# slothfulxtx/Texture-GS

Hardware: AMD Instinct MI355X
Metric: fwd+bwd views/sec @800x800, 300k Gaussians + 1024^2 texture; HBM GB/s vs roofline (higher is better)
Workload: dtype f32; 1 GPU; c3: N=300000 Gaussians, cubemap 6x1024x1024x3 f32, 800x800, fwd+bwd, sh_degree 3; parallelism=views sharded dp1, view_pipeline=3 HIP streams, order=accumulate, forwards begun one view per stream ahead, grad_allreduce=none (1 GPU)

## Files before the change

### include/texgs.h

```cpp
#ifndef TEXGS_H
#define TEXGS_H

#include <stddef.h>
#include <stdint.h>

#ifdef __cplusplus
extern "C" {
#endif

#define TEXGS_ABI_VERSION 19
#define TEXGS_TILE 16
#define TEXGS_REC_TEST_FLOATS 8
#define TEXGS_REC_SHADE_FLOATS 20
#define TEXGS_ACC_FLOATS 32

typedef struct TexGSFrame {
    int32_t image_height;
    int32_t image_width;
    float   tanfovx;
    float   tanfovy;
    float   scale_modifier;
    int32_t sh_degree;
    int32_t sh_coeffs;
    int32_t tex_res;
// ... 33 lines not shown
typedef struct TexGSBinning {
    uint32_t  num_rendered;
    uint64_t* keys_unsorted;
    uint64_t* keys_sorted;
    uint32_t* point_list;
    uint32_t* ranges;
    uint32_t* tile_order;
    void*     sort_temp;
    size_t    sort_temp_bytes;
} TexGSBinning;

typedef struct TexGSImage {
    float*    out_color;
    float*    out_depth;
    float*    out_norm;
    float*    out_alpha;
    float*    final_T;
    uint32_t* n_contrib;
    uint32_t* tex_bin_count;
    uint32_t* survivors;
    uint16_t* surv_qmask;
    uint32_t* surv_count;
    uint32_t* tex_bin_resv;
} TexGSImage;
#define TEXGS_RESV_WORDS 192

#define TEXGS_ACC_MEANS3D 1
#define TEXGS_ACC_MEANS2D 2
#define TEXGS_ACC_SHS 4
#define TEXGS_ACC_OPACITIES 8
#define TEXGS_ACC_SCALES 16
#define TEXGS_ACC_ROTATIONS 32
#define TEXGS_ACC_UVS 64
#define TEXGS_ACC_COLOR_OFFSET 128
#define TEXGS_ACC_COV3D 256
#define TEXGS_ACC_ALL 511

#define TEXGS_WANT_TEXTURE   1
#define TEXGS_WANT_GAUSSIANS 2
#define TEXGS_WANT_ALL       3

typedef struct TexGSGrads {
    const float* dL_dcolor;
    const float* dL_ddepth;
    const float* dL_dnorm;
    const float* dL_dalpha;
    float* acc;
    float* dL_dmeans3D;
// ... 190 lines not shown
```

### texture-gs_amd/csrc/render.hip

```cpp
#include "common.h"
#include "wave_ops.h"
#include "texrec_math.h"

namespace {

typedef unsigned long long ull;

struct __attribute__((packed, aligned(4))) Texel3 { float x, y, z; };
__device__ __forceinline__ Texel3 load_texel(const float* __restrict__ tex, uint32_t boff) {
    return *reinterpret_cast<const Texel3*>(reinterpret_cast<const char*>(tex) + boff);
}

typedef uint32_t tg_u4 __attribute__((ext_vector_type(4)));
template <class T> __device__ __forceinline__ T nt_load(const T* p) {
    return __builtin_nontemporal_load(p);
}
template <class T> __device__ __forceinline__ void nt_store(T* p, T v) {
    __builtin_nontemporal_store(v, p);
}
__device__ __forceinline__ uint2 nt_load2(const uint2* p) {
    const unsigned long long v = nt_load(reinterpret_cast<const unsigned long long*>(p));
    return make_uint2((uint32_t)v, (uint32_t)(v >> 32));
}
__device__ __forceinline__ void nt_store2(uint2* p, uint2 v) {
// ... 53 lines not shown
        return ah * dx * dx + bh * dx * dy + ch * dy * dy;
    };
    auto edge_y = [&](float dy) {
        const float dx = fminf(dx1, fmaxf(dx0, bh * dy * iha));
        return ah * dx * dx + bh * dx * dy + ch * dy * dy;
    };
    const float best = fmaxf(fmaxf(edge_x(dx0), edge_x(dx1)), fmaxf(edge_y(dy0), edge_y(dy1)));
    return best >= thr - 1e-3f * fabsf(thr) - 1e-4f;
}

struct PixArgs {
    int W, H, tiles_x, num_tiles, R;
    const uint2* ranges;
    const uint32_t* tile_order;
    const uint32_t* point_list;
    const float4* rec_test;
    const float4* rec_shade;
    const float* texture;
    const float* bg;
    uint2*    surv;
    uint16_t* surv_qm;
    uint32_t* surv_cnt;
    uint32_t* resv;
};

__device__ __forceinline__ bool wave_block(const PixArgs& a, int& tile, int& wave) {
    const int b = (int)blockIdx.x, k = b >> 3;
    wave = k & 3;
    const int rank = ((k >> 2) << 3) | (b & 7);
    if (rank >= a.num_tiles) return false;
    tile = (int)a.tile_order[rank];
    return true;
}
inline int blend_grid(int num_tiles) { return 4 * ((num_tiles + 7) & ~7); }

#define TG_BALLOT(P) __builtin_amdgcn_ballot_w64((bool)(P))
__device__ __forceinline__ int mbcnt64(ull m) {
    return (int)__builtin_amdgcn_mbcnt_hi((uint32_t)(m >> 32), __builtin_amdgcn_mbcnt_lo((uint32_t)m, 0u));
}

__device__ __forceinline__ uint32_t tap_bin(const CubeTap& ct, int nb) { return (uint32_t)((ct.face * nb + (ct.y0 >> 5)) * nb + (ct.x0 >> 5)); }
__device__ __forceinline__ bool tap_binned(const CubeTap& ct) { return ct.dox != 0u && ct.doy != 0u; }
#define TG_RESV 64
#define TG_RESV_EMPTY 0xFFFFFFFFu
#define TG_SLOT_NONE 0xFFFFFFFFu
#define TG_SLOT_OVF  0x80000000u
__device__ __forceinline__ int tap_home(const CubeTap& ct) { return ((ct.x0 >> 5) & 7) | (((ct.y0 >> 5) & 7) << 3); }
template <class P> __device__ __forceinline__ uint32_t& resv_bin(P& p, int h) { return reinterpret_cast<uint32_t*>(&p.B[h])[3]; }

#define TG_RING 128
#define TG_DUMMY 64
struct Planes {
    float4 A[65];
    float4 B[65];
    float4 C[65];
    float4 D[65];
    float4 E[65];
    float4 F[65];
    float2 G[66];
};

#define KEY_J(K)   ((int)((K) & 127u))
#define KEY_PL(K)  ((int)(((K) >> 8) & 63u))
#define KEY_OX(K)  ((int)(((K) >> 14) & 7u))
#define KEY_OY(K)  ((int)(((K) >> 17) & 7u))

__device__ __forceinline__ void lane_pixel(int lane, int& ox, int& oy) {
    ox = (((lane >> 4) & 1) << 2) | (lane & 3);
    oy = (((lane >> 5) & 1) << 2) | ((lane >> 2) & 3);
}

__device__ __forceinline__ void load_chunk(const PixArgs& a, Planes& P, int lane, bool live, uint32_t id, uint32_t pos,
                                           float4& T0, float4& T1) {
    const float4 z = make_float4(0.f, 0.f, 0.f, 0.f);
    float4 S0 = z, S1 = z, S2 = z, S3 = z, S4 = z;
    T0 = z; T1 = make_float4(0.f, 0.f, -1.f, 1.f);
    if (live) {
        const float4* __restrict__ tp = a.rec_test + 2 * (size_t)id;
        const float4* __restrict__ sp = a.rec_shade + (TEXGS_REC_SHADE_FLOATS / 4) * (size_t)id;
        T0 = tp[0]; T1 = tp[1]; S0 = sp[0]; S1 = sp[1]; S2 = sp[2]; S3 = sp[3]; S4 = sp[4];
    }
    P.A[lane] = T0;
    { float* pb = reinterpret_cast<float*>(&P.B[lane]); pb[0] = T1.x; pb[1] = T1.y; pb[2] = __uint_as_float(pos); }
    P.C[lane] = make_float4(S3.z, S3.w, S4.x, S4.y);
    P.D[lane] = S0; P.E[lane] = S1; P.F[lane] = S2;
    P.G[lane] = make_float2(S3.x, S3.y);
}
__device__ __forceinline__ void init_dummy(Planes& P, int lane) {
    if (lane == 0) {
        const float4 z = make_float4(0.f, 0.f, 0.f, 0.f);
        P.A[TG_DUMMY] = z; P.B[TG_DUMMY] = make_float4(0.f, 0.f, __uint_as_float(0xFFFFFFFFu), 0.f); P.C[TG_DUMMY] = z;
        P.D[TG_DUMMY] = z; P.E[TG_DUMMY] = z; P.F[TG_DUMMY] = z; P.G[TG_DUMMY] = make_float2(0.f, 0.f);
    }
}

#define FQ_CAP 128
struct __attribute__((aligned(16))) FwdLds {
    Planes p;
    uint2 q[FQ_CAP];
    ull col[64 * 3];
    uint32_t ring[TG_RING];
    uint8_t list[4][64];
    uint32_t ccnt[TG_RESV / 2];
// ... 127 lines not shown
            const float4 t0 = nt0, t1 = nt1;
            r += 64;
            nt0 = zt0; nt1 = zt1;
            if (r + lane < todo) {
                const float4* __restrict__ tp = a.rec_test + 2 * (size_t)nid;
                nt0 = tp[0]; nt1 = tp[1];
            }
            nid = (r + 64 + lane < todo) ? a.point_list[range.x + r + 64 + lane] : 0u;
            const bool reach = block_reachable(t0.x, t0.y, t0.z, t0.w, t1.x, t1.w, t1.z, wpx, wpy, 7.0f);
            const ull m = TG_BALLOT(reach);
            if (reach) L.ring[(qh + nq + mbcnt64(m)) & (TG_RING - 1)] = (uint32_t)idx;
            nq += __popcll(m);
        }
        if (nq == 0) break;
        const int take = min(64, nq);
        __builtin_amdgcn_wave_barrier();
        uint32_t pos = 0xFFFFFFFFu, id = 0u;
        if (lane < take) {
            pos = L.ring[(qh + lane) & (TG_RING - 1)];
            id = a.point_list[range.x + pos];
        }
        qh = (qh + take) & (TG_RING - 1); nq -= take;
        float4 T0, T1;
        load_chunk(a, L.p, lane, lane < take, id, pos, T0, T1);
        reinterpret_cast<uint32_t*>(&L.list[0][0])[lane] = 0x40404040u;
        __builtin_amdgcn_wave_barrier();
        int len[4];
        uint32_t qbits = 0u;
#pragma unroll
        for (int q = 0; q < 4; ++q) {
            const bool rowdone = ((done_mask >> (16 * q)) & 0xFFFFull) == 0xFFFFull;
            const bool geo = (lane < take) &&
                block_reachable(T0.x, T0.y, T0.z, T0.w, T1.x, T1.w, T1.z, wpx + (float)((q & 1) << 2), wpy + (float)((q >> 1) << 2), 3.0f);
            qbits |= geo ? (1u << q) : 0u;
            const bool rq = geo && !rowdone;
            const ull m = TG_BALLOT(rq);
            len[q] = __popcll(m);
            if (rq) L.list[q][mbcnt64(m)] = (uint8_t)lane;
        }
        if (a.surv != nullptr) {
            if (lane < take) { nt_store2(a.surv + sbase + nsurv + lane, make_uint2(id, pos)); nt_store(a.surv_qm + sbase + nsurv + lane, (uint16_t)qbits); }
            nsurv += take;
        }
        __builtin_amdgcn_wave_barrier();
        int tmax = max(max(len[0], len[1]), max(len[2], len[3]));
        auto test_one = [&](const float4& A, const float4& B, const float4& Cc, const int j) -> bool {
                const float power = gauss_power(A.z, A.w, B.x, A.x - pxf, A.y - pyf);
// ... 105 lines not shown
using texrec_math::rec_word0;
using texrec_math::rec_pack;
using texrec_math::rec_unpack;
__device__ __forceinline__ void rec_store(uint32_t* __restrict__ base, uint32_t slot, const Rec4 r) {
    tg_u4 v; v.x = r.a; v.y = r.b; v.z = r.c; v.w = r.d;
    __builtin_nontemporal_store(v, reinterpret_cast<tg_u4*>(base) + slot);
}
__device__ __forceinline__ Rec4 rec_load(const Rec4* __restrict__ p) {
    const tg_u4 v = __builtin_nontemporal_load(reinterpret_cast<const tg_u4*>(p));
    Rec4 r; r.a = v.x; r.b = v.y; r.c = v.z; r.d = v.w;
    return r;
}

#define TG_MOMENTS_ALL  0x0FFFFFFFu
#define TG_MOMENTS_NOUV (0x3Fu | (0x7Fu << 21))

#ifdef K7_TRACE
#define K7_TRACE_BLOCKS 32768
__device__ unsigned long long k7_trace[4 * K7_TRACE_BLOCKS];
#endif
namespace k7_occ {
#define BQ_CAP 64
#define K7_GATHER 1
#define K7_WAVES_PER_SIMD 4
#include "render_bwd_body.h"
#undef BQ_CAP
#undef K7_GATHER
#undef K7_WAVES_PER_SIMD
}
namespace k7_lds {
#define BQ_CAP 128
#define K7_GATHER 0
#define K7_WAVES_PER_SIMD 2
#include "render_bwd_body.h"
#undef BQ_CAP
#undef K7_GATHER
#undef K7_WAVES_PER_SIMD
}

__global__ void __launch_bounds__(1024)
k_bin_offsets(int nbins, const uint32_t* __restrict__ count, uint32_t* __restrict__ base, uint32_t* __restrict__ cursor,
              uint32_t* __restrict__ order, uint32_t* __restrict__ stats) {
    constexpr int BO_MAX = 32;
    __shared__ uint32_t s_w[16];
    __shared__ uint32_t s_carry;
    const int tid = (int)threadIdx.x, lane = tid & 63, wv = tid >> 6;
    if (tid == 0) s_carry = 0u;
    __syncthreads();
    for (int c0 = 0; c0 < nbins; c0 += 1024 * BO_MAX) {
        const int n = min(nbins - c0, 1024 * BO_MAX);
        const int per = (n + 1023) >> 10;
        const int i0 = c0 + tid * per;
        uint32_t v[BO_MAX];
        uint32_t sum = 0u;
#pragma unroll
        for (int k = 0; k < BO_MAX; ++k) { v[k] = (k < per && i0 + k < c0 + n) ? count[i0 + k] + count[nbins + i0 + k] : 0u; sum += v[k]; }
        uint32_t incl = sum;
#pragma unroll
        for (int d = 1; d < 64; d <<= 1) { const uint32_t o = (uint32_t)__shfl_up((int)incl, d, 64); if (lane >= d) incl += o; }
// ... 99 lines not shown
            if (y >= R || xq >= R * 3) continue;
            unsafeAtomicAdd(dtex + ((size_t)(face * R + y) * R) * 3 + xq, texrec_math::from_fixed(q, down));
        }
        __syncthreads();
    }
}

inline PixArgs make_pix(const CamConst& c, const TexGSFrame* f, const TexGSInputs* in, const TexGSGeom* g,
                        const TexGSBinning* b, const TexGSImage* img) {
    PixArgs a;
    a.W = c.W; a.H = c.H; a.tiles_x = c.tiles_x; a.num_tiles = c.tiles_x * c.tiles_y; a.R = c.R;
    a.ranges = reinterpret_cast<const uint2*>(b->ranges);
    a.point_list = b->point_list;
    a.tile_order = b->tile_order;
    a.rec_test = reinterpret_cast<const float4*>(g->rec_test);
    a.rec_shade = reinterpret_cast<const float4*>(g->rec_shade);
    a.texture = in->texture;
    a.bg = f->bg;
    const bool hand = img->survivors != nullptr && img->surv_qmask != nullptr && img->surv_count != nullptr;
    a.surv = hand ? reinterpret_cast<uint2*>(img->survivors) : nullptr;
    a.surv_qm = hand ? img->surv_qmask : nullptr;
    a.surv_cnt = hand ? img->surv_count : nullptr;
    a.resv = img->tex_bin_resv;
    return a;
}

inline TexBinArgs make_bins(const CamConst& c, const TexGSImage* img, const TexGSGrads* gr) {
    TexBinArgs tb;
    tb.nb = (c.R + 31) >> 5;
    const bool on = (gr->want & TEXGS_WANT_TEXTURE) && img->tex_bin_count != nullptr && img->tex_bin_resv != nullptr && gr->tex_bins != nullptr &&
                    gr->tex_bin_cursor != nullptr && gr->tex_bin_base != nullptr && gr->tex_rec_cap > 0;
    tb.rec = on ? reinterpret_cast<uint32_t*>(gr->tex_bins) : nullptr;
    tb.cursor = on ? gr->tex_bin_cursor : nullptr;
    tb.base = on ? gr->tex_bin_base : nullptr;
    tb.order = on ? gr->tex_bin_base + tex_bin_count(c.R) + 1 : nullptr;
    tb.stats = on ? gr->tex_bin_cursor + tex_bin_count(c.R) : nullptr;
    tb.cap = on ? gr->tex_rec_cap : 0u;
    return tb;
}

}

size_t tex_bin_count(int R) {
    const size_t nb = (size_t)((R + 31) >> 5);
    return 6 * nb * nb;
}
// ... 4 lines not shown
    if (in->texture)
        hipLaunchKernelGGL(k_render_fwd<true>, dim3(blend_grid(a.num_tiles)), dim3(64), 0, s, a, img->out_color, img->out_depth,
                           img->out_norm, img->out_alpha, img->final_T, img->n_contrib, img->tex_bin_resv ? img->tex_bin_count : (uint32_t*)nullptr);
    else
        hipLaunchKernelGGL(k_render_fwd<false>, dim3(blend_grid(a.num_tiles)), dim3(64), 0, s, a, img->out_color, img->out_depth,
                           img->out_norm, img->out_alpha, img->final_T, img->n_contrib, (uint32_t*)nullptr);
    return hipGetLastError();
}

hipError_t launch_render_bwd(const CamConst& c, const TexGSFrame* f, const TexGSInputs* in, const TexGSGeom* g,
                       const TexGSBinning* b, const TexGSImage* img, TexGSGrads* gr, hipStream_t s) {
    const PixArgs a = make_pix(c, f, in, g, b, img);
    const TexBinArgs tb = make_bins(c, img, gr);
    const bool taps = in->texture != nullptr;
    const bool tex = taps && (gr->want & TEXGS_WANT_TEXTURE) && gr->dL_dtexture != nullptr;
    const bool geo = (gr->want & TEXGS_WANT_GAUSSIANS) != 0;
    if (!tex && !geo) return hipSuccess;
    if (tex && tb.rec)
        hipLaunchKernelGGL(k_bin_offsets, dim3(1), dim3(1024), 0, s, (int)tex_bin_count(c.R), (const uint32_t*)img->tex_bin_count,
                           gr->tex_bin_base, gr->tex_bin_cursor, gr->tex_bin_base + tex_bin_count(c.R) + 1, tb.stats);
    const dim3 grid(blend_grid(a.num_tiles)), blk(64);
#define K7_LAUNCH(NS, TEX, GEO, UVG, TAPS) hipLaunchKernelGGL((NS::k_render_bwd<TEX, GEO, UVG, TAPS>), grid, blk, 0, s, a, tb, img->final_T, \
        img->n_contrib, gr->dL_dcolor, gr->dL_ddepth, gr->dL_dnorm, gr->dL_dalpha, gr->acc, gr->dL_dtexture)
    if (!taps)            K7_LAUNCH(k7_occ, false, true, false, false);
    else if (tex && geo)  K7_LAUNCH(k7_occ, true, true, true, true);
    else if (tex)         K7_LAUNCH(k7_lds, true, false, false, true);
    else                  K7_LAUNCH(k7_occ, false, true, true, true);
#undef K7_LAUNCH
    return hipGetLastError();
}

bool tex_bins_enabled(const CamConst& c, const TexGSInputs* in, const TexGSImage* img, const TexGSGrads* gr) {
    return in->texture != nullptr && gr->dL_dtexture != nullptr && make_bins(c, img, gr).rec != nullptr;
}

hipError_t launch_texgrad_reduce(const CamConst& c, const TexGSImage* img, TexGSGrads* gr, hipStream_t s) {
    const TexBinArgs tb = make_bins(c, img, gr);
    if (!tb.rec) return hipSuccess;
    hipLaunchKernelGGL(k_texgrad_reduce, dim3((unsigned)tex_bin_count(c.R)), dim3(TB_THREADS), 0, s, c.R, tb, gr->dL_dtexture);
    return hipGetLastError();
}

#ifdef K7_TRACE
extern "C" __attribute__((visibility("default"))) int texgs_debug_k7_trace(void* host_dst) {
    return (int)hipMemcpyFromSymbol(host_dst, HIP_SYMBOL(k7_trace), sizeof(unsigned long long) * 4 * K7_TRACE_BLOCKS);
}
#endif
```

### texture-gs_amd/csrc/render_bwd_body.h

```cpp
#if K7_GATHER
struct PlanesT { float4 A[65]; float4 B[65]; };
#else
typedef Planes PlanesT;
#endif
struct __attribute__((aligned(16))) BwdLds {
    float4 items[BQ_CAP * 3 + 3];
    float4 abuf[BQ_CAP];
    PlanesT p;
    float4 dpix[64];
    float4 dgeo[64];
    uint32_t task[64];
    uint8_t list[4][64];
    uint32_t tpos[TG_RESV], tend[TG_RESV];
};

template <bool TEX, bool GEO, bool UVG, bool TAPS>
__global__ void __launch_bounds__(64, K7_WAVES_PER_SIMD)
k_render_bwd(PixArgs a, TexBinArgs tb, const float* __restrict__ final_T, const uint32_t* __restrict__ n_contrib,
             const float* __restrict__ dL_dcolor, const float* __restrict__ dL_ddepth,
             const float* __restrict__ dL_dnorm, const float* __restrict__ dL_dalpha,
             float* __restrict__ acc, float* __restrict__ dtex) {
    static_assert(TAPS || (!TEX && !UVG), "no texture: no texture gradient and no UV chain");
    static_assert(GEO || !UVG, "the UV chain ends in the per-Gaussian moments");
    static_assert(TEX || GEO, "nothing to compute");
// ... 67 lines not shown
    uint2 nsv = make_uint2(0u, 0xFFFFFFFFu);
    uint32_t nqm = 0u;
    if (ns - 1 - lane >= 0) { nsv = nt_load2(a.surv + sbase + (ns - 1 - lane)); nqm = nt_load(a.surv_qm + sbase + (ns - 1 - lane)); }
    struct Seg { int n_items, n_it; uint32_t it_lo, it_hi, it_first; };
    struct Round {
        bool have;
        int e, pl, jj, axis;
        uint32_t key;
        uint32_t slot;
        uint32_t ovf0, ovf1;
        uint32_t fxw, fyw;
        uint32_t o00, dox, doy;
        float w, vd0, vd1, vd2, nu0, nu1, nu2, inv;
        float T, araw;
        float fx, fy, ka, kb, kc, kd;
        Texel3 t00, t01, t10, t11;
#if K7_GATHER
        float4 sd, se, sf;
        float4 c5;
#endif
    };
    uint32_t cid = 0u;
    (void)cid;
    auto front_a = [&](int rbase, Round& R, int n_items) {
        R.e = rbase + lane;
        R.have = R.e < n_items;
        float4 it = make_float4(1.f, 0.f, 0.f, 0.f);
        if (R.have) {
            it = L.abuf[R.e];
        }
        R.key = __float_as_uint(it.w);
        R.pl = KEY_PL(R.key);
        R.jj = KEY_J(R.key);
        if constexpr (GEO) { R.T = it.x; R.araw = it.z; }
        else R.w = fminf(TG_ALPHA_MAX, it.z) * it.x;
#if K7_GATHER
        const float4* __restrict__ sp = a.rec_shade + (TEXGS_REC_SHADE_FLOATS / 4) * (size_t)(uint32_t)__builtin_amdgcn_ds_bpermute(R.jj << 2, (int)cid);
        if constexpr (TAPS) { R.sd = sp[0]; R.se = sp[1]; }
        R.sf = sp[2];
        const float4 s3 = sp[3];
        const float2 s4 = *reinterpret_cast<const float2*>(sp + 4);
        R.vd1 = s3.x; R.vd2 = s3.y;
        R.c5 = make_float4(s3.z, s3.w, s4.x, s4.y);
#endif
    };
    auto front_b = [&](Round& R) {
        const uint32_t key = R.key;
        const int jj = R.jj;
#if K7_GATHER
        const float4 f_ = R.sf;
        R.vd0 = f_.w;
#else
        const float4 f_ = L.p.F[jj];
        const float2 g2 = L.p.G[jj];
        R.vd0 = f_.w; R.vd1 = g2.x; R.vd2 = g2.y;
#endif
        if constexpr (TAPS) {
            const float2 xy = *reinterpret_cast<const float2*>(&L.p.A[jj]);
#if K7_GATHER
            const float4 d_ = R.sd, e4 = R.se;
// ... 99 lines not shown
                const uint32_t p1 = (uint32_t)__builtin_amdgcn_ds_bpermute(ldr, (int)R.ovf1);
                if (ovf) { const uint32_t pos = p0 + (slot & 63u); slot = (pos < p1) ? pos : TG_SLOT_NONE; }
            }
            if (slot < tb.cap) {
                rec_store(tb.rec, slot, rec_pack(R.fxw, R.fyw >> 10, (int)(R.fyw & 31u), (int)((R.fyw >> 5) & 31u), x0, x1, x2));
            } else if (R.have && (x0 != 0.f || x1 != 0.f || x2 != 0.f)) {
                scatter_direct(dtex, R.o00, R.dox, R.doy, R.fx, R.fy, x0, x1, x2);
            }
        }
    };
    for (int hi = ns; hi > 0; hi -= 64) {
        if (hi > 128) __builtin_amdgcn_s_setprio(3); else if (hi > 64) __builtin_amdgcn_s_setprio(2); else __builtin_amdgcn_s_setprio(0);
        const bool live = hi - 1 - lane >= 0;
        const uint32_t id = nsv.x, pos = nsv.y, qm = nqm;
        nsv = make_uint2(0u, 0xFFFFFFFFu); nqm = 0u;
        if (hi - 65 - lane >= 0) { nsv = nt_load2(a.surv + sbase + (hi - 65 - lane)); nqm = nt_load(a.surv_qm + sbase + (hi - 65 - lane)); }
        const int take = min(64, hi);
        if ((int)__builtin_amdgcn_readlane((int)pos, take - 1) >= wave_last) continue;
        __builtin_amdgcn_wave_barrier();
        cid = id;
#if K7_GATHER
        {
            float4 T0 = make_float4(0.f, 0.f, 0.f, 0.f), T1 = make_float4(0.f, 0.f, -1.f, 1.f);
            if (live) { const float4* __restrict__ tp = a.rec_test + 2 * (size_t)id; T0 = tp[0]; T1 = tp[1]; }
            L.p.A[lane] = T0;
            float* pb = reinterpret_cast<float*>(&L.p.B[lane]); pb[0] = T1.x; pb[1] = T1.y; pb[2] = __uint_as_float(pos);
        }
#else
        float4 T0, T1;
        load_chunk(a, L.p, lane, live, id, pos, T0, T1);
#endif
        reinterpret_cast<uint32_t*>(&L.list[0][0])[lane] = 0x40404040u;
        __builtin_amdgcn_wave_barrier();
        int len[4];
#pragma unroll
        for (int q = 0; q < 4; ++q) {
            const bool rq = live && ((int)pos < rowlast[q]) && ((qm >> q) & 1u);
            const ull m = TG_BALLOT(rq);
            len[q] = __popcll(m);
            if (rq) L.list[q][mbcnt64(m)] = (uint8_t)lane;
        }
        __builtin_amdgcn_wave_barrier();
        const int tmax = max(max(len[0], len[1]), max(len[2], len[3]));
        int t = 0;
        auto stage_a = [&](Seg& sg) {
            sg.n_it = 0; sg.n_items = 0; sg.it_lo = 0u; sg.it_hi = 0u; sg.it_first = 0u;
            auto test_one = [&](const float4& cA, const float4& cB, const int cj) -> bool {
// ... 186 lines not shown
```

### texture-gs_amd/texgs/_lib.py

```python
import contextlib
import ctypes as C
import os

_HERE = os.path.dirname(os.path.abspath(__file__))
LIB_PATH = os.environ.get("TEXGS_LIB") or os.path.join(os.path.dirname(_HERE), "libtexgs.so")

ABI_VERSION = 19
TILE = 16
REC_TEST_FLOATS = 8
REC_SHADE_FLOATS = 20
TEXBIN_RECORD_FLOATS = 4
RESV_WORDS = 192
ACC_FLOATS = 32
WANT_TEXTURE, WANT_GAUSSIANS, WANT_ALL = 1, 2, 3

_fp = C.c_void_p


class Frame(C.Structure):
    _fields_ = [("image_height", C.c_int32), ("image_width", C.c_int32), ("tanfovx", C.c_float),
                ("tanfovy", C.c_float), ("scale_modifier", C.c_float), ("sh_degree", C.c_int32),
                ("sh_coeffs", C.c_int32), ("tex_res", C.c_int32), ("num_gaussians", C.c_int32),
                ("debug", C.c_int32), ("bg", _fp), ("viewmatrix", _fp), ("projmatrix", _fp), ("campos", _fp)]


class Inputs(C.Structure):
    _fields_ = [("means3D", _fp), ("shs", _fp), ("opacities", _fp), ("scales", _fp), ("rotations", _fp),
                ("uvs", _fp), ("gradient_uvs", _fp), ("texture", _fp), ("color_offset", _fp), ("cov3D_precomp", _fp)]


class Geom(C.Structure):
    _fields_ = [("rec_test", _fp), ("rec_shade", _fp), ("depth", _fp), ("radii", _fp), ("rect", _fp), ("tiles_touched", _fp),
                ("offsets", _fp), ("scan_temp", _fp), ("scan_temp_bytes", C.c_size_t)]


class Binning(C.Structure):
    _fields_ = [("num_rendered", C.c_uint32), ("keys_unsorted", _fp), ("keys_sorted", _fp), ("point_list", _fp),
                ("ranges", _fp), ("tile_order", _fp), ("sort_temp", _fp), ("sort_temp_bytes", C.c_size_t)]


class Image(C.Structure):
    _fields_ = [("out_color", _fp), ("out_depth", _fp), ("out_norm", _fp), ("out_alpha", _fp),
                ("final_T", _fp), ("n_contrib", _fp), ("tex_bin_count", _fp),
                ("survivors", _fp), ("surv_qmask", _fp), ("surv_count", _fp), ("tex_bin_resv", _fp)]


class Grads(C.Structure):
    _fields_ = [("dL_dcolor", _fp), ("dL_ddepth", _fp), ("dL_dnorm", _fp), ("dL_dalpha", _fp), ("acc", _fp),
                ("dL_dmeans3D", _fp), ("dL_dmeans2D", _fp), ("dL_dshs", _fp), ("dL_dopacities", _fp),
                ("dL_dscales", _fp), ("dL_drotations", _fp), ("dL_duvs", _fp), ("dL_dtexture", _fp),
                ("dL_dcolor_offset", _fp), ("dL_dcov3D", _fp), ("want", C.c_uint32), ("tex_bins", _fp), ("tex_bin_cursor", _fp), ("tex_bin_base", _fp),
                ("tex_rec_cap", C.c_uint32),
                ("accumulate", C.c_int32), ("dL_dvd_residue", _fp)]


class UVNetStruct(C.Structure):
    _fields_ = [(n, _fp) for n in ("W1", "b1", "W2", "b2", "emb", "W3", "b3", "W4", "b4", "W5", "b5", "xyz_offset", "xyz_scale")] \
        + [("hidden", C.c_int32)]


class HashGridStruct(C.Structure):
    _fields_ = [("n_levels", C.c_int32), ("n_features", C.c_int32), ("log2_hashmap_size", C.c_int32), ("base_resolution", C.c_float),
                ("per_level_scale", C.c_float)]


HASHGRID_MAX_LEVELS = 16
HASHGRID_FEATURES = 4
# ... 184 lines not shown
```

### texture-gs_amd/texgs/rasterizer.py

```python
import ctypes as C
import math
import os as _os
import threading as _threading
import weakref as _weakref
from collections import namedtuple
from types import SimpleNamespace
from typing import NamedTuple

import torch
from torch import nn

from . import _lib

USE_TEX_BINS = _os.environ.get("TEXGS_TEX_BINS", "1") != "0"
TEX_REC_CAP = int(_os.environ.get("TEXGS_REC_CAP", "0"))
DIRECT_LEAF_GRADS = _os.environ.get("TEXGS_DIRECT_LEAF_GRADS", "0") != "0"
TEX_REC_BYTES_MAX = int(float(_os.environ.get("TEXGS_BIN_GB_MAX", "4")) * (1 << 30))
_ACC_BITS = dict(means3D=1, means2D=2, shs=4, opacities=8, scales=16, rotations=32, uvs=64, color_offset=128, cov3D=256)


class GaussianRasterizationSettings(NamedTuple):
    image_height: int
    image_width: int
    tanfovx: float
    tanfovy: float
    bg: torch.Tensor
    scale_modifier: float
    viewmatrix: torch.Tensor
    projmatrix: torch.Tensor
    sh_degree: int
    campos: torch.Tensor
    prefiltered: bool
    debug: bool


_ptr = _lib.ptr


def _f32c(t: torch.Tensor, name: str, device) -> torch.Tensor:
    if not isinstance(t, torch.Tensor):
# ... 203 lines not shown
def _pin_take(words):
    pool = _PIN_POOL.setdefault(words, [])
    return pool.pop() if pool else torch.empty(max(words, 1), dtype=torch.int32).pin_memory()


def _pin_give(t):
    pool = _PIN_POOL.setdefault(t.numel(), [])
    if len(pool) < 16:
        pool.append(t)


def _prefetch_take(device, key):
    skey = (device.index, int(torch.cuda.current_stream(device).cuda_stream))
    lst = _PREFETCH.get(skey, ())
    for k, (key_k, fwd) in enumerate(lst):
        if key_k == key:
            del lst[k]
            if not lst:
                del _PREFETCH[skey]
            return fwd


_Args = namedtuple("_Args", "means3D shs opacities scales rotations uvs gradient_uvs texture color_offset cov3D_precomp N K R")
_HANDOFF = tuple(n for n, _ in _lib.Image._fields_[6:])


def _check_inputs(st, means3D, shs, opacities, scales, rotations, uvs, gradient_uvs, texture, color_offset=None, cov3D_precomp=None):
    device = means3D.device
    N = means3D.shape[0]
    means3D = _f32c(means3D, "means3D", device)
    if means3D.dim() != 2 or means3D.shape[1] != 3:
        raise ValueError("means3D must be [N,3]")
    opacities = _f32c(opacities, "opacities", device)
    if opacities.numel() != N:
        raise ValueError(f"per-Gaussian inputs must have exactly N rows (N={N}; opacities {tuple(opacities.shape)})")
    if cov3D_precomp is not None:
        if texture is not None:
            raise ValueError("cov3D_precomp is an input of the untextured surface only")
        cov3D_precomp = _f32c(cov3D_precomp, "cov3D_precomp", device)
        if cov3D_precomp.shape != (N, 6):
            raise ValueError(f"cov3D_precomp must be [N,6], got {tuple(cov3D_precomp.shape)}")
        scales = rotations = None
    else:
        scales = _f32c(scales, "scales", device)
        rotations = _f32c(rotations, "rotations", device)
        if scales.shape != (N, 3) or rotations.shape != (N, 4):
            raise ValueError("per-Gaussian inputs must have exactly N rows "
# ... 19 lines not shown
        K = shs.shape[1]
        if K > 15:
            raise ValueError("shs holds at most 15 view-dependent coefficients (degree 3)")
    if color_offset is not None:
        color_offset = _f32c(color_offset, "color_offset", device)
        if color_offset.shape != (N, 3):
            raise ValueError(f"color_offset must be [N,3], got {tuple(color_offset.shape)}")
    if int(st.sh_degree) < 0 or int(st.sh_degree) > 3:
        raise ValueError("sh_degree must be in [0,3]")
    return _Args(means3D, shs, opacities, scales, rotations, uvs, gradient_uvs, texture, color_offset, cov3D_precomp, N, K, R)


def _add_handoff(ar, cap, tiles, R, want_counts):
    if cap is not None:
        ar.add("survivors", (4 * max(cap, 1), 2), torch.int32)
        ar.add("surv_qmask", (4 * max(cap, 1),), torch.int16)
    if tiles is not None:
        ar.add("surv_count", (4 * tiles,), torch.int32)
        if want_counts:
            ar.add("tex_bin_count", (2 * int(_lib.load().texgs_tex_bin_count(R)),), torch.int32)
            ar.add("tex_bin_resv", (4 * tiles, _lib.RESV_WORDS), torch.int32)


class _Forward:

    def __init__(self, st, tensors, for_backward, count_bins, lazy):
        self.st, self.raw, self.flags = st, tensors, (for_backward, count_bins, lazy)

    def key(self):
        t = lambda x: None if x is None else (x.data_ptr(), x._version, tuple(x.shape), x.requires_grad)
        st = self.st
        return (int(st.image_height), int(st.image_width), float(st.tanfovx), float(st.tanfovy), float(st.scale_modifier), int(st.sh_degree),
                bool(st.debug), t(st.bg), t(st.viewmatrix), t(st.projmatrix), t(st.campos)) + tuple(t(x) for x in self.raw) + self.flags

    def begin(self):
        lib = _lib.load()
        self._plan()
        a, N, stream = self.args, self.args.N, self.stream
        with torch.cuda.device(a.means3D.device):
            self.fix.commit()
            self._bind()
            refs = self.refs
            _lib.call(lib.texgs_preprocess_forward, *refs, stream)
            pin = self.pin = _pin_take(int(lib.texgs_num_rendered_words(N)))
            _lib.call(lib.texgs_num_rendered_begin, refs[2], N, pin.data_ptr(), pin.numel(), 0, stream)
            self.d_ev = torch.cuda.Event()
# ... 60 lines not shown
        self.binning = self.bin_ar = None
        if entry is None and not batched:
            self._alloc_bin(self.cap, fix)
        self.refs = [C.byref(x) for x in (self.frame, self.inputs, self.geom)]

    def _add_lists(self, ar):
        ar.add("ranges", (self.tiles, 2), torch.int32)
        ar.add("tile_order", (self.tiles,), torch.int32)
        if self.handoff:
            _add_handoff(ar, None, self.tiles, self.args.R, self.want_counts)

    def _alloc_bin(self, cap, lists_ar, commit=True):
        c1, tiles = max(cap, 1), self.tiles
        sort_bytes = _lib.load().texgs_sort_temp_bytes(cap, tiles)
        ar = self.bin_ar = _Arena(self.fix.device)
        ar.add("keys_unsorted", (c1,), torch.int64)
        ar.add("keys_sorted", (c1,), torch.int64)
        ar.add("point_list", (c1,), torch.int32)
        ar.add("sort_temp", (sort_bytes,), torch.uint8)
        if lists_ar is None:
            self._add_lists(ar)
        if self.handoff:
            _add_handoff(ar, cap, None, self.args.R, self.want_counts)
        self.sort_bytes = sort_bytes
        if commit:
            ar.commit()
            self._bind_bin(lists_ar)
        return ar

    def _bind_bin(self, lists_ar):
        ar, sort_bytes = self.bin_ar, self.sort_bytes
        la = lists_ar if lists_ar is not None else ar
        self.binning = _lib.Binning(0, ar.ptr("keys_unsorted"), ar.ptr("keys_sorted"), ar.ptr("point_list"), la.ptr("ranges"),
                                    la.ptr("tile_order"), ar.ptr("sort_temp"), sort_bytes)
        for n in _HANDOFF:
            setattr(self.img, n, (ar if n in ar.specs else la).ptr(n))

    def finish(self):
        lib, a, img, entry, refs = _lib.load(), self.args, self.img, self.entry, self.refs
        for_backward, _, lazy = self.flags
        stream, cap, pin = self.stream, self.cap, self.pin
        if self.binned is not None:
            D, fp, ready = self.binned
            shared, binning = False, self.binning
            with torch.cuda.device(a.means3D.device):
                cur = torch.cuda.current_stream(a.means3D.device)
                if cur.cuda_stream != stream:
                    cur.wait_event(ready)
                from .multiview import views_entries
                _lib.call(views_entries().render_forward_binned, *refs, C.byref(binning), C.byref(img), cur.cuda_stream)
            return self._finished(binning, D, cap, shared, fp)
        with torch.cuda.device(a.means3D.device):
            self.d_ev.synchronize()
            d_host, fp_host = C.c_uint32(0), C.c_uint64(0)
            _lib.call(lib.texgs_num_rendered_reduce, pin.data_ptr(), a.N, C.byref(d_host), C.byref(fp_host))
            _pin_give(pin)
            D, fp = int(d_host.value), int(fp_host.value)
            shared = entry is not None and fp == entry.fingerprint and D == entry.D
            if shared:
# ... 9 lines not shown
                if entry is not None:
                    cap = max(cap, grown)
                    self._alloc_bin(cap, None)
                    _lib.call(lib.texgs_depth_sort_scan, refs[2], a.N, stream)
                elif D > cap:
                    cap = grown
                    self._alloc_bin(cap, self.fix)
                binning = self.binning
                binning.num_rendered = D
                _lib.call(lib.texgs_bin_sort_render_forward, *refs, C.byref(binning), C.byref(img), stream)
                _CAPACITY_HINT[self.hint_key] = max(_CAPACITY_HINT.get(self.hint_key, 0), grown)
                if GEOM_CACHE:
                    _GEOM[self.gkey] = _GeomEntry(
                        self.gints, self.cam_key, fp, D, cap, tuple(getattr(binning, n) for n, _ in _lib.Binning._fields_[1:]),
                        (self.fix, self.bin_ar), (img.survivors, img.surv_qmask, img.surv_count) if self.handoff else None,
                        (img.tex_bin_count, img.tex_bin_resv) if (self.handoff and img.tex_bin_count) else None)
        return self._finished(binning, D, cap, shared, fp)

    def _finished(self, binning, D, cap, shared, fp):
        a, img, entry = self.args, self.img, self.entry
        for_backward, _, lazy = self.flags
        arenas = (self.fix,) + ((self.bin_ar,) if self.bin_ar is not None else ()) + (tuple(entry.arenas) if shared else ())
        tensors = _Tensors(arenas, keep=self.keep, radii=self.outs[4], for_backward=bool(for_backward))
        for n in _HANDOFF:
            if getattr(img, n) is None:
                tensors[n] = None
        state = _State(self.frame, self.inputs, self.geom, binning, img, tensors, a, D, cap, self.tiles, self.want_counts,
                       bool(lazy and for_backward), shared)
        state.fingerprint = fp
        return self.outs, state

    def abandon(self):
        if self.binned is not None:
            return
        self.d_ev.synchronize()
        _pin_give(self.pin)


_BATCH_SCOPE = None


class _Request:
    __slots__ = ("fwd", "stream", "batched")

    def __init__(self, fwd, stream):
        self.fwd, self.stream, self.batched = fwd, stream, False

# ... 156 lines not shown
    fwd = _Forward(st, (means3D, shs, opacities, scales, rotations, uvs, gradient_uvs, texture, color_offset, cov3D_precomp),
                   for_backward, count_bins, lazy)
    if _BATCH_SCOPE is not None:
        _BATCH_SCOPE.requests.append(_Request(fwd, torch.cuda.current_stream(device)))
        return
    _register_begun(fwd.begin(), limit=4)


def forward_raw(st, means3D, shs, opacities, scales, rotations, uvs, gradient_uvs, texture, color_offset=None,
                for_backward=True, cov3D_precomp=None, count_bins=None, lazy=False):
    _gpu_only(means3D.device)
    fwd = _Forward(st, (means3D, shs, opacities, scales, rotations, uvs, gradient_uvs, texture, color_offset, cov3D_precomp),
                   for_backward, count_bins, lazy)
    pend = _prefetch_take(means3D.device, fwd.key()) if _PREFETCH else None
    return (pend or fwd.begin()).finish()


def _late_handoff(s: _State):
    lib = _lib.load()
    device = s.args.means3D.device
    stream = torch.cuda.current_stream(device).cuda_stream
    ar = _Arena(device)
    _add_handoff(ar, s.cap, s.tiles, s.R, s.want_counts)
    ar.add("scratch_out", (8, s.H, s.W), torch.float32)
    ar.add("final_T", (s.H, s.W), torch.float32)
    ar.add("n_contrib", (s.H, s.W), torch.int32)
    ar.commit()
    so = ar.ptr("scratch_out")
    hw = 4 * s.H * s.W
    img = _lib.Image(so, so + 3 * hw, so + 4 * hw, so + 7 * hw, ar.ptr("final_T"), ar.ptr("n_contrib"), *(ar.ptr(n) for n in _HANDOFF))
    _lib.call(lib.texgs_render_forward, C.byref(s.frame), C.byref(s.inputs), C.byref(s.geom), C.byref(s.bin), C.byref(img), stream)
    s.tensors._arenas = tuple(s.tensors._arenas) + (ar,)
    for n in _HANDOFF:
        setattr(s.img, n, ar.ptr(n))
        s.tensors.pop(n, None)
        if n not in ar.specs:
            s.tensors[n] = None
    _GEOM_STATS["late_handoffs"] += 1


def _plan_outputs(N, K, textured, has_cov, has_coff, want, sinks, device):
    shapes = {}
    if want & _lib.WANT_GAUSSIANS:
        shapes = dict(means3D=(N, 3), means2D=(N, 3), opacities=(N, 1))
        if has_cov:
            shapes["cov3D"] = (N, 6)
        else:
            shapes.update(scales=(N, 3), rotations=(N, 4))
        if textured:
            shapes["uvs"] = (N, 3)
        if K > 0:
            shapes["shs"] = (N, K, 3)
        if has_coff:
            shapes["color_offset"] = (N, 3)
    fresh = [n for n in shapes if n not in sinks]
    sizes = [math.prod(shapes[n]) for n in fresh]
    flat = torch.empty(sum(sizes), dtype=torch.float32, device=device).split(sizes) if fresh else ()
    outs, mask = {n: v.view(shapes[n]) for n, v in zip(fresh, flat)}, 0
    for n in shapes.keys() - set(fresh):
        t = outs[n] = sinks[n]
# ... 227 lines not shown
```

Before: 1070 views/s.

## Stream survivor Gaussian records from forward to backward as contiguous rows

```diff
diff --git a/include/texgs.h b/include/texgs.h
--- a/include/texgs.h
+++ b/include/texgs.h
@@ -79,8 +79,10 @@
     uint16_t* surv_qmask;
     uint32_t* surv_count;
     uint32_t* tex_bin_resv;
+    float*    surv_rec;
 } TexGSImage;
 #define TEXGS_RESV_WORDS 192
+#define TEXGS_SURV_ROW_FLOATS 24
 
 #define TEXGS_ACC_MEANS3D 1
 #define TEXGS_ACC_MEANS2D 2
diff --git a/texture-gs_amd/csrc/render.hip b/texture-gs_amd/csrc/render.hip
--- a/texture-gs_amd/csrc/render.hip
+++ b/texture-gs_amd/csrc/render.hip
@@ -99,6 +99,7 @@
     uint16_t* surv_qm;
     uint32_t* surv_cnt;
     uint32_t* resv;
+    float4*   surv_rec;
 };
 
 __device__ __forceinline__ bool wave_block(const PixArgs& a, int& tile, int& wave) {
@@ -136,6 +137,12 @@
     float4 F[65];
     float2 G[66];
 };
+#define TG_SURV_ROW (TEXGS_SURV_ROW_FLOATS / 4)
+static_assert(TEXGS_SURV_ROW_FLOATS == 24, "surv_row_store and K7's row offsets state the 96-byte row");
+__device__ __forceinline__ void surv_row_store(float4* __restrict__ row, const float4& T0, const float4& T1, const float4& S0,
+                                               const float4& S1, const float4& S2, const float4& S3, const float4& S4) {
+    row[0] = T0; row[1] = S0; row[2] = S1; row[3] = S2; row[4] = S3; row[5] = make_float4(S4.x, S4.y, T1.x, T1.y);
+}
 
 #define KEY_J(K)   ((int)((K) & 127u))
 #define KEY_PL(K)  ((int)(((K) >> 8) & 63u))
@@ -148,7 +155,7 @@
 }
 
 __device__ __forceinline__ void load_chunk(const PixArgs& a, Planes& P, int lane, bool live, uint32_t id, uint32_t pos,
-                                           float4& T0, float4& T1) {
+                                           float4& T0, float4& T1, float4* __restrict__ row = nullptr) {
     const float4 z = make_float4(0.f, 0.f, 0.f, 0.f);
     float4 S0 = z, S1 = z, S2 = z, S3 = z, S4 = z;
     T0 = z; T1 = make_float4(0.f, 0.f, -1.f, 1.f);
@@ -156,6 +163,7 @@
         const float4* __restrict__ tp = a.rec_test + 2 * (size_t)id;
         const float4* __restrict__ sp = a.rec_shade + (TEXGS_REC_SHADE_FLOATS / 4) * (size_t)id;
         T0 = tp[0]; T1 = tp[1]; S0 = sp[0]; S1 = sp[1]; S2 = sp[2]; S3 = sp[3]; S4 = sp[4];
+        if (row != nullptr) surv_row_store(row, T0, T1, S0, S1, S2, S3, S4);
     }
     P.A[lane] = T0;
     { float* pb = reinterpret_cast<float*>(&P.B[lane]); pb[0] = T1.x; pb[1] = T1.y; pb[2] = __uint_as_float(pos); }
@@ -329,7 +337,8 @@
         }
         qh = (qh + take) & (TG_RING - 1); nq -= take;
         float4 T0, T1;
-        load_chunk(a, L.p, lane, lane < take, id, pos, T0, T1);
+        load_chunk(a, L.p, lane, lane < take, id, pos, T0, T1,
+                   a.surv_rec != nullptr ? a.surv_rec + TG_SURV_ROW * (sbase + (size_t)(nsurv + lane)) : nullptr);
         reinterpret_cast<uint32_t*>(&L.list[0][0])[lane] = 0x40404040u;
         __builtin_amdgcn_wave_barrier();
         int len[4];
@@ -481,19 +490,34 @@
 namespace k7_occ {
 #define BQ_CAP 64
 #define K7_GATHER 1
+#define K7_STREAM 0
 #define K7_WAVES_PER_SIMD 4
 #include "render_bwd_body.h"
 #undef BQ_CAP
 #undef K7_GATHER
+#undef K7_STREAM
+#undef K7_WAVES_PER_SIMD
+}
+namespace k7_str {
+#define BQ_CAP 64
+#define K7_GATHER 1
+#define K7_STREAM 1
+#define K7_WAVES_PER_SIMD 4
+#include "render_bwd_body.h"
+#undef BQ_CAP
+#undef K7_GATHER
+#undef K7_STREAM
 #undef K7_WAVES_PER_SIMD
 }
 namespace k7_lds {
 #define BQ_CAP 128
 #define K7_GATHER 0
+#define K7_STREAM 0
 #define K7_WAVES_PER_SIMD 2
 #include "render_bwd_body.h"
 #undef BQ_CAP
 #undef K7_GATHER
+#undef K7_STREAM
 #undef K7_WAVES_PER_SIMD
 }
 
@@ -639,6 +663,7 @@
     a.surv_qm = hand ? img->surv_qmask : nullptr;
     a.surv_cnt = hand ? img->surv_count : nullptr;
     a.resv = img->tex_bin_resv;
+    a.surv_rec = hand ? reinterpret_cast<float4*>(img->surv_rec) : nullptr;
     return a;
 }
 
@@ -689,10 +714,11 @@
     const dim3 grid(blend_grid(a.num_tiles)), blk(64);
 #define K7_LAUNCH(NS, TEX, GEO, UVG, TAPS) hipLaunchKernelGGL((NS::k_render_bwd<TEX, GEO, UVG, TAPS>), grid, blk, 0, s, a, tb, img->final_T, \
         img->n_contrib, gr->dL_dcolor, gr->dL_ddepth, gr->dL_dnorm, gr->dL_dalpha, gr->acc, gr->dL_dtexture)
-    if (!taps)            K7_LAUNCH(k7_occ, false, true, false, false);
-    else if (tex && geo)  K7_LAUNCH(k7_occ, true, true, true, true);
+    const bool str = a.surv_rec != nullptr;
+    if (!taps)            { if (str) K7_LAUNCH(k7_str, false, true, false, false); else K7_LAUNCH(k7_occ, false, true, false, false); }
+    else if (tex && geo)  { if (str) K7_LAUNCH(k7_str, true, true, true, true);    else K7_LAUNCH(k7_occ, true, true, true, true); }
     else if (tex)         K7_LAUNCH(k7_lds, true, false, false, true);
-    else                  K7_LAUNCH(k7_occ, false, true, true, true);
+    else                  { if (str) K7_LAUNCH(k7_str, false, true, true, true);   else K7_LAUNCH(k7_occ, false, true, true, true); }
 #undef K7_LAUNCH
     return hipGetLastError();
 }
diff --git a/texture-gs_amd/csrc/render_bwd_body.h b/texture-gs_amd/csrc/render_bwd_body.h
--- a/texture-gs_amd/csrc/render_bwd_body.h
+++ b/texture-gs_amd/csrc/render_bwd_body.h
@@ -1,3 +1,6 @@
+#if K7_STREAM && !K7_GATHER
+#error "the survivor stream replaces the gathers of the K7_GATHER configuration"
+#endif
 #if K7_GATHER
 struct PlanesT { float4 A[65]; float4 B[65]; };
 #else
@@ -113,6 +116,10 @@
     };
     uint32_t cid = 0u;
     (void)cid;
+#if K7_STREAM
+    const char* __restrict__ srow = reinterpret_cast<const char*>(a.surv_rec + TG_SURV_ROW * sbase);
+    int chi = 0;
+#endif
     auto front_a = [&](int rbase, Round& R, int n_items) {
         R.e = rbase + lane;
         R.have = R.e < n_items;
@@ -126,7 +133,11 @@
         if constexpr (GEO) { R.T = it.x; R.araw = it.z; }
         else R.w = fminf(TG_ALPHA_MAX, it.z) * it.x;
 #if K7_GATHER
+#if K7_STREAM
+        const float4* __restrict__ sp = reinterpret_cast<const float4*>(srow + (uint32_t)(chi - 1 - R.jj) * (uint32_t)(16 * TG_SURV_ROW)) + 1;
+#else
         const float4* __restrict__ sp = a.rec_shade + (TEXGS_REC_SHADE_FLOATS / 4) * (size_t)(uint32_t)__builtin_amdgcn_ds_bpermute(R.jj << 2, (int)cid);
+#endif
         if constexpr (TAPS) { R.sd = sp[0]; R.se = sp[1]; }
         R.sf = sp[2];
         const float4 s3 = sp[3];
@@ -272,7 +283,17 @@
 #if K7_GATHER
         {
             float4 T0 = make_float4(0.f, 0.f, 0.f, 0.f), T1 = make_float4(0.f, 0.f, -1.f, 1.f);
+#if K7_STREAM
+            chi = hi;
+            if (live) {
+                const float4* __restrict__ tp = reinterpret_cast<const float4*>(srow + (uint32_t)(hi - 1 - lane) * (uint32_t)(16 * TG_SURV_ROW));
+                T0 = tp[0];
+                const float2 t1 = *reinterpret_cast<const float2*>(reinterpret_cast<const float*>(tp + TG_SURV_ROW - 1) + 2);
+                T1.x = t1.x; T1.y = t1.y;
+            }
+#else
             if (live) { const float4* __restrict__ tp = a.rec_test + 2 * (size_t)id; T0 = tp[0]; T1 = tp[1]; }
+#endif
             L.p.A[lane] = T0;
             float* pb = reinterpret_cast<float*>(&L.p.B[lane]); pb[0] = T1.x; pb[1] = T1.y; pb[2] = __uint_as_float(pos);
         }
diff --git a/texture-gs_amd/texgs/_lib.py b/texture-gs_amd/texgs/_lib.py
--- a/texture-gs_amd/texgs/_lib.py
+++ b/texture-gs_amd/texgs/_lib.py
@@ -10,6 +10,7 @@
 REC_TEST_FLOATS = 8
 REC_SHADE_FLOATS = 20
 TEXBIN_RECORD_FLOATS = 4
+SURV_ROW_FLOATS = 24
 RESV_WORDS = 192
 ACC_FLOATS = 32
 WANT_TEXTURE, WANT_GAUSSIANS, WANT_ALL = 1, 2, 3
@@ -42,7 +43,7 @@
 class Image(C.Structure):
     _fields_ = [("out_color", _fp), ("out_depth", _fp), ("out_norm", _fp), ("out_alpha", _fp),
                 ("final_T", _fp), ("n_contrib", _fp), ("tex_bin_count", _fp),
-                ("survivors", _fp), ("surv_qmask", _fp), ("surv_count", _fp), ("tex_bin_resv", _fp)]
+                ("survivors", _fp), ("surv_qmask", _fp), ("surv_count", _fp), ("tex_bin_resv", _fp), ("surv_rec", _fp)]
 
 
 class Grads(C.Structure):
diff --git a/texture-gs_amd/texgs/rasterizer.py b/texture-gs_amd/texgs/rasterizer.py
--- a/texture-gs_amd/texgs/rasterizer.py
+++ b/texture-gs_amd/texgs/rasterizer.py
@@ -16,6 +16,7 @@
 TEX_REC_CAP = int(_os.environ.get("TEXGS_REC_CAP", "0"))
 DIRECT_LEAF_GRADS = _os.environ.get("TEXGS_DIRECT_LEAF_GRADS", "0") != "0"
 TEX_REC_BYTES_MAX = int(float(_os.environ.get("TEXGS_BIN_GB_MAX", "4")) * (1 << 30))
+SURV_REC_BYTES_MAX = int(float(_os.environ.get("TEXGS_SURV_REC_GB_MAX", "1")) * (1 << 30))
 _ACC_BITS = dict(means3D=1, means2D=2, shs=4, opacities=8, scales=16, rotations=32, uvs=64, color_offset=128, cov3D=256)
 
 
@@ -265,7 +266,8 @@
 
 
 _Args = namedtuple("_Args", "means3D shs opacities scales rotations uvs gradient_uvs texture color_offset cov3D_precomp N K R")
-_HANDOFF = tuple(n for n, _ in _lib.Image._fields_[6:])
+_HANDOFF = tuple(n for n, _ in _lib.Image._fields_[6:11])
+_STREAM = _lib.Image._fields_[11][0]
 
 
 def _check_inputs(st, means3D, shs, opacities, scales, rotations, uvs, gradient_uvs, texture, color_offset=None, cov3D_precomp=None):
@@ -331,6 +333,14 @@
             ar.add("tex_bin_resv", (4 * tiles, _lib.RESV_WORDS), torch.int32)
 
 
+def _add_stream(ar, cap):
+    rows = 4 * max(cap, 1)
+    fits = 4 * rows * _lib.SURV_ROW_FLOATS <= SURV_REC_BYTES_MAX
+    if fits:
+        ar.add(_STREAM, (rows, _lib.SURV_ROW_FLOATS), torch.float32)
+    return fits
+
+
 class _Forward:
 
     def __init__(self, st, tensors, for_backward, count_bins, lazy):
@@ -437,6 +447,7 @@
             self._add_lists(ar)
         if self.handoff:
             _add_handoff(ar, cap, None, self.args.R, self.want_counts)
+            _add_stream(ar, cap)
         self.sort_bytes = sort_bytes
         if commit:
             ar.commit()
@@ -450,6 +461,7 @@
                                     la.ptr("tile_order"), ar.ptr("sort_temp"), sort_bytes)
         for n in _HANDOFF:
             setattr(self.img, n, (ar if n in ar.specs else la).ptr(n))
+        setattr(self.img, _STREAM, ar.ptr(_STREAM))
 
     def finish(self):
         lib, a, img, entry, refs = _lib.load(), self.args, self.img, self.entry, self.refs
@@ -505,7 +517,7 @@
         for_backward, _, lazy = self.flags
         arenas = (self.fix,) + ((self.bin_ar,) if self.bin_ar is not None else ()) + (tuple(entry.arenas) if shared else ())
         tensors = _Tensors(arenas, keep=self.keep, radii=self.outs[4], for_backward=bool(for_backward))
-        for n in _HANDOFF:
+        for n in _HANDOFF + (_STREAM,):
             if getattr(img, n) is None:
                 tensors[n] = None
         state = _State(self.frame, self.inputs, self.geom, binning, img, tensors, a, D, cap, self.tiles, self.want_counts,
@@ -708,13 +720,15 @@
     stream = torch.cuda.current_stream(device).cuda_stream
     ar = _Arena(device)
     _add_handoff(ar, s.cap, s.tiles, s.R, s.want_counts)
+    _add_stream(ar, s.cap)
     ar.add("scratch_out", (8, s.H, s.W), torch.float32)
     ar.add("final_T", (s.H, s.W), torch.float32)
     ar.add("n_contrib", (s.H, s.W), torch.int32)
     ar.commit()
     so = ar.ptr("scratch_out")
     hw = 4 * s.H * s.W
-    img = _lib.Image(so, so + 3 * hw, so + 4 * hw, so + 7 * hw, ar.ptr("final_T"), ar.ptr("n_contrib"), *(ar.ptr(n) for n in _HANDOFF))
+    img = _lib.Image(so, so + 3 * hw, so + 4 * hw, so + 7 * hw, ar.ptr("final_T"), ar.ptr("n_contrib"), *(ar.ptr(n) for n in _HANDOFF),
+                     ar.ptr(_STREAM))
     _lib.call(lib.texgs_render_forward, C.byref(s.frame), C.byref(s.inputs), C.byref(s.geom), C.byref(s.bin), C.byref(img), stream)
     s.tensors._arenas = tuple(s.tensors._arenas) + (ar,)
     for n in _HANDOFF:
@@ -722,6 +736,8 @@
         s.tensors.pop(n, None)
         if n not in ar.specs:
             s.tensors[n] = None
+    setattr(s.img, _STREAM, ar.ptr(_STREAM))
+    s.tensors.pop(_STREAM, None)
     _GEOM_STATS["late_handoffs"] += 1
 
 
```

New measurement: 1036 views/s. -3.2%, worse.
